# MarcioCerqueira/RealTimeDepthDiffusion

Hardware: AMD Instinct MI355X
Metric: Mpixel-iterations/s (solver sweep) (higher is better)
Workload: dtype f32

## Files before the change

### realtimedepthdiffusion_amd/csrc/persist_sync.hpp

```cpp
#pragma once
#include <hip/hip_runtime.h>

namespace rtdd {

constexpr int kSyncStatus = 0, kSyncWithhold = 1, kSyncLimit = 2, kSyncNonLocal = 3 , kSyncFailedSeq = 4,
              kSyncConfirmPtr = 6 , kSyncWild = 8, kSyncFlags = 32, kSyncMaxTiles = 1024, kSyncFlagStride = 64;
constexpr int kSyncWords = kSyncFlags + kSyncMaxTiles * kSyncFlagStride;
constexpr unsigned long long kDefaultPollLimit = 20000000ull;
constexpr unsigned long long kArrivalPollLimit = 150000ull;

constexpr float kWildDepth = 0x1p100f;

#ifdef __HIPCC__
__device__ __forceinline__ bool depth_is_wild(float d) { return !(__builtin_fabsf(d) < kWildDepth); }
__device__ __forceinline__ int load_wild_word(const int *sync_words) { return sync_words[kSyncWild]; }
__device__ __forceinline__ bool solve_is_dead(int *sync_words, int seq, bool first) {
    if (!sync_words) return false;
    if (__hip_atomic_load(&sync_words[kSyncStatus], __ATOMIC_RELAXED, __HIP_MEMORY_SCOPE_AGENT) == 0) {
        if (first && seq != 0) {
            int *confirm = *(int *const *)(sync_words + kSyncConfirmPtr);
            if (confirm) __hip_atomic_store(confirm, seq, __ATOMIC_RELAXED, __HIP_MEMORY_SCOPE_SYSTEM);
        }
        return false;
    }
    if (first && __hip_atomic_load(&sync_words[kSyncFailedSeq], __ATOMIC_RELAXED, __HIP_MEMORY_SCOPE_AGENT) == 0)
        __hip_atomic_store(&sync_words[kSyncFailedSeq], seq, __ATOMIC_RELAXED, __HIP_MEMORY_SCOPE_AGENT);
    return true;
}

__device__ __forceinline__ int exchange_poll_offset(int tid, int bx, int by, int gx, int gy, int tile_base) {
    const int pw = tid >> 6, pl = tid & 63;
    if (pw != 0 || pl >= 9 || pl == 4) return -1;
    const int nx = bx + pl % 3 - 1, ny = by + pl / 3 - 1;
    if (nx < 0 || ny < 0 || nx >= gx || ny >= gy) return -1;
    return (kSyncFlags + (tile_base + ny * gx + nx) * kSyncFlagStride) * (int)sizeof(int);
}

__device__ __forceinline__ int load_flag_at(const int *base, unsigned off) {
    int v;
    asm volatile("global_load_dword %0, %1, %2 sc1\n\ts_waitcnt vmcnt(0)" : "=v"(v) : "v"(off), "s"(base) : "memory");
    return v;
}

template <bool ACQUIRE = true, bool ARRIVAL = false>
__device__ __forceinline__ bool exchange_wait_at(int *sync_words, int *dead_lds, int tid, int tile_id, int poll_off, int value, int tile_base = 0) {
    int *flags = sync_words + kSyncFlags + tile_base * kSyncFlagStride;
    if (tid == 0 && __hip_atomic_load(&sync_words[kSyncWithhold], __ATOMIC_RELAXED, __HIP_MEMORY_SCOPE_AGENT) != tile_id + 1)
        __hip_atomic_store(&flags[tile_id * kSyncFlagStride], value, __ATOMIC_RELAXED, __HIP_MEMORY_SCOPE_AGENT);
    if (poll_off >= 0) {
        unsigned long long t0 = 0, limit = 0;
        unsigned spins = 0;
        while (load_flag_at(sync_words, (unsigned)poll_off) - value < 0) {
            __builtin_amdgcn_s_sleep(4);
            if ((++spins & 63u) == 0) {
                const unsigned long long now = __builtin_amdgcn_s_memrealtime();
                if (t0 == 0) {
                    t0 = now;
                    const int l = __hip_atomic_load(&sync_words[kSyncLimit], __ATOMIC_RELAXED, __HIP_MEMORY_SCOPE_AGENT);
                    limit = l > 0 ? (unsigned long long)l : kDefaultPollLimit;
                    if (ARRIVAL && limit > kArrivalPollLimit) limit = kArrivalPollLimit;
                }
                const bool failed = __hip_atomic_load(&sync_words[kSyncStatus], __ATOMIC_RELAXED, __HIP_MEMORY_SCOPE_AGENT) != 0;
                if (failed || now - t0 > limit) {
                    if (!failed) __hip_atomic_store(&sync_words[kSyncStatus], 1, __ATOMIC_RELAXED, __HIP_MEMORY_SCOPE_AGENT);
                    __hip_atomic_store(dead_lds, 1, __ATOMIC_RELAXED, __HIP_MEMORY_SCOPE_WORKGROUP);
                    break;
                }
            }
        }
    }
    if (ACQUIRE && tid < 64) { __builtin_amdgcn_fence(__ATOMIC_ACQUIRE, "agent"); asm volatile("s_waitcnt vmcnt(0)" ::: "memory"); }
    if (!ACQUIRE && tid < 64) asm volatile("s_waitcnt vmcnt(0)" ::: "memory");
    __syncthreads();
    return __hip_atomic_load(dead_lds, __ATOMIC_RELAXED, __HIP_MEMORY_SCOPE_WORKGROUP) != 0;
}

template <bool ACQUIRE = true, bool ARRIVAL = false>
__device__ __forceinline__ bool exchange_wait(int *sync_words, int *dead_lds, int tid, int tile_id, int bx, int by, int gx, int gy, int value, int tile_base = 0) {
    return exchange_wait_at<ACQUIRE, ARRIVAL>(sync_words, dead_lds, tid, tile_id, exchange_poll_offset(tid, bx, by, gx, gy, tile_base), value, tile_base);
}

#endif

}
```

### realtimedepthdiffusion_amd/csrc/rbgs_blocked.hip

```cpp
#include <type_traits>

#include "rtdd_internal.hpp"
#include "persist_sync.hpp"
#include "sweep_common.hpp"

namespace rtdd {
namespace {

__device__ __forceinline__ float from_prev_lane(float v) {
    return __int_as_float(__builtin_amdgcn_update_dpp(0, __float_as_int(v), 0x138, 0xF, 0xF, true));
}
__device__ __forceinline__ float from_next_lane(float v) {
    return __int_as_float(__builtin_amdgcn_update_dpp(0, __float_as_int(v), 0x130, 0xF, 0xF, true));
}
__device__ __forceinline__ float div3(float n, float d, float y) {
    const float q0 = n * y;
    const float r = __builtin_fmaf(-d, q0, n);
    return __builtin_fmaf(r, y, q0);
}


__device__ __forceinline__ void store_sc1(float4 *p, float4 v) {
    typedef float f4v __attribute__((ext_vector_type(4)));
    const f4v t = {v.x, v.y, v.z, v.w};
// ... 58 lines not shown
            wr[g][i] = (in && x0 + i + 1 < cols) ? lut[mv[i] & 255] : 0.0f;
            wd[g][i] = (in && y + 1 < rows) ? lut[(mv[i] >> 8) & 255] : 0.0f;
            if (!in || (mv[i] & kMetaDirichlet)) dirichlet |= 1u << (g * 4 + i);
        }
        const float w = from_prev_lane(wr[g][3]);
        wl0[g] = (lx > 0 && x0 > 0) ? w : 0.0f;
    }
    {
        const int y = y0 - 1;
        uint4 m = make_uint4(0, 0, 0, 0);
        const bool ok = colok && y >= 0 && y + 1 < rows;
        if (ok) m = *(const uint4 *)(M + (size_t)y * ip + x0);
        const uint32_t mv[4] = {m.x, m.y, m.z, m.w};
#pragma unroll
        for (int i = 0; i < 4; i++) wu0[i] = (ok && x0 + i < cols) ? lut[(mv[i] >> 8) & 255] : 0.0f;
    }
#pragma unroll
    for (int g = 0; g < G; g++)
#pragma unroll
        for (int i = 0; i < 4; i++) {
            const float wl = i == 0 ? wl0[g] : wr[g][i - 1];
            const float wu = g == 0 ? wu0[i] : wd[g - 1][i];
            float c = 0.0f;
            c += wl; c += wr[g][i]; c += wu; c += wd[g][i];
            cnt[g][i] = c == 0.0f ? 1.0f : c;
            rcp[g][i] = rcp_rn(cnt[g][i]);
            unsafe |= cnt[g][i] < 0x1p-126f;
        }
    const bool wave_unsafe = __builtin_amdgcn_ballot_w64(unsafe) != 0 || wild_word == wild_seq;

    constexpr uint32_t kTinyT = 2u * 0x0D800000u - 1u;
    const int wv = tid >> 6, nwv = (int)blockDim.x >> 6;
    const int flag_idx = (tid & 63) == 0 ? (wv > 0 ? wv - 1 : wv) : (wv < nwv - 1 ? wv + 1 : wv);
    auto publish = [&](int h, int buf) {
        *(f4r *)&edge[buf][tr][0][lx] = a[0];
        *(f4r *)&edge[buf][tr][1][lx] = a[G - 1];
        __hip_atomic_store(&published[wv], h + 1, __ATOMIC_RELEASE, __HIP_MEMORY_SCOPE_WORKGROUP);
    };
    auto half = [&](int h, auto fast, auto col, bool last_of_block) {
        constexpr bool FAST = decltype(fast)::value;
        constexpr int C = decltype(col)::value;
        for (;;) {
            const int f = __hip_atomic_load(&published[flag_idx], __ATOMIC_RELAXED, __HIP_MEMORY_SCOPE_WORKGROUP);
            if (__builtin_amdgcn_ballot_w64(f < h + 1) == 0) break;
            __builtin_amdgcn_s_sleep(1);
        }
        __builtin_amdgcn_fence(__ATOMIC_ACQUIRE, "workgroup");
        float4 up4 = edge[C][tr > 0 ? tr - 1 : 0][tr > 0 ? 1 : 0][lx];
        float4 dn4 = edge[C][tr < ntr - 1 ? tr + 1 : tr][tr < ntr - 1 ? 0 : 1][lx];
        if (!FAST) { if (tr == 0) up4 = make_float4(0, 0, 0, 0); if (tr == ntr - 1) dn4 = make_float4(0, 0, 0, 0); }
        const float up[4] = {up4.x, up4.y, up4.z, up4.w}, dn[4] = {dn4.x, dn4.y, dn4.z, dn4.w};
        float xl0[G], xr3[G];
        auto wsum = [&](int g, int i) {
            const float xl = i == 0 ? xl0[g] : a[g][i - 1];
            const float xr = i == 3 ? xr3[g] : a[g][i + 1];
            const float xu = g == 0 ? up[i] : a[g - 1][i];
            const float xd = g == G - 1 ? dn[i] : a[g + 1][i];
            const float wl = i == 0 ? wl0[g] : wr[g][i - 1];
            const float wu = g == 0 ? wu0[i] : wd[g - 1][i];
            float sum = 0.0f;
            sum = CONTRACT ? __builtin_fmaf(wl, xl, sum) : sum + wl * xl;
            sum = CONTRACT ? __builtin_fmaf(wr[g][i], xr, sum) : sum + wr[g][i] * xr;
            sum = CONTRACT ? __builtin_fmaf(wu, xu, sum) : sum + wu * xu;
            sum = CONTRACT ? __builtin_fmaf(wd[g][i], xd, sum) : sum + wd[g][i] * xd;
            return sum;
        };
        auto group = [&](auto pick) {
            float q[G][4];
            uint32_t tmin = 0xFFFFFFFFu;
#pragma unroll
            for (int g = 0; g < G; g++) {
                if (!pick(g)) continue;
                if (((g + 0) & 1) == C) { xl0[g] = from_prev_lane(a[g][3]); if (!FAST && lx == 0) xl0[g] = 0.0f; }
                if (((g + 3) & 1) == C) { xr3[g] = from_next_lane(a[g][0]); if (!FAST && lx == LX - 1) xr3[g] = 0.0f; }
#pragma unroll
                for (int i = 0; i < 4; i++) {
                    if (((g + i) & 1) != C) continue;
                    const float sum = wsum(g, i);
                    if (FAST) { q[g][i] = div3(sum, cnt[g][i], rcp[g][i]); tmin = min(tmin, (__float_as_uint(sum) << 1) + 0xFFFFFFFFu); }
                    else q[g][i] = sum / cnt[g][i];
                }
            }
            if (FAST && __builtin_expect(__builtin_amdgcn_ballot_w64(tmin < kTinyT) != 0, 0)) {
                bool suspect = false;
#pragma unroll
                for (int g = 0; g < G; g++) {
                    if (!pick(g)) continue;
#pragma unroll
                    for (int i = 0; i < 4; i++) {
                        if (((g + i) & 1) != C) continue;
                        bool s;
                        q[g][i] = div_tiny(wsum(g, i), cnt[g][i], rcp[g][i], s);
                        suspect |= s;
                    }
                }
                if (__builtin_expect(__builtin_amdgcn_ballot_w64(suspect) != 0, 0)) {
#pragma unroll
                    for (int g = 0; g < G; g++) {
                        if (!pick(g)) continue;
#pragma unroll
                        for (int i = 0; i < 4; i++) if (((g + i) & 1) == C) q[g][i] = wsum(g, i) / cnt[g][i];
                    }
                }
            }
#pragma unroll
            for (int g = 0; g < G; g++) {
                if (!pick(g)) continue;
#pragma unroll
                for (int i = 0; i < 4; i++) {
                    if (((g + i) & 1) != C) continue;
                    const float x = a[g][i];
                    float r = __builtin_amdgcn_fmed3f(q[g][i], 0.0f, 255.0f);
                    if (SOR) { r = CONTRACT ? __builtin_fmaf(omega, r - x, x) : x + omega * (r - x); r = __builtin_amdgcn_fmed3f(r, 0.0f, 255.0f); }
                    a[g][i] = (dirichlet >> (g * 4 + i)) & 1u ? x : r;
                }
            }
        };
        __builtin_amdgcn_s_setprio(1);
        group([](int g) { return g == 0 || g == G - 1; });
        if (!last_of_block) publish(h + 1, C ^ 1);
        __builtin_amdgcn_s_setprio(0);
        group([](int g) { return g != 0 && g != G - 1; });
    };

    const int tile_id = by * gx + bx;
    int h = 0, s = 0, blk = 0;
    for (;; blk++) {
        const int s_end = min(s + block_sweeps, nsweeps);
        publish(h, 0);
        using C0 = std::integral_constant<int, 0>; using C1 = std::integral_constant<int, 1>;
        for (; s < s_end; s++) {
            if (!wave_unsafe) { half(h, std::true_type{}, C0{}, false); half(h + 1, std::true_type{}, C1{}, s + 1 >= s_end); }
            else { half(h, std::false_type{}, C0{}, false); half(h + 1, std::false_type{}, C1{}, s + 1 >= s_end); }
            h += 2;
        }
        if (!PERSIST || s >= nsweeps) break;
        float *Ex = (blk & 1) ? X : Y;
        int tid_x = tid;
        asm volatile("" : "+v"(tid_x));
        const int lx = tid_x % LX, tr = tid_x / LX;
        const int x0 = bx * TW - hx + 4 * lx, y0 = by * TH - hy + tr * G;
        const bool colok = x0 >= 0 && x0 < cols;
        const bool xin = colok && 4 * lx >= hx && 4 * lx < EW - hx;
#pragma unroll
        for (int g = 0; g < G; g++) {
            const int y = y0 + g, ty = tr * G + g;
            const bool central = xin && ty >= hy && ty < eh - hy && y < rows;
            const bool band = ty < 2 * hy || ty >= eh - 2 * hy || 4 * lx < 2 * hx || 4 * lx >= EW - 2 * hx;
            if (central && band) store_sc1((float4 *)(Ex + (size_t)y * ip + x0), make_float4(a[g][0], a[g][1], a[g][2], a[g][3]));
        }
        asm volatile("s_waitcnt vmcnt(0)" ::: "memory");
        __syncthreads();
#ifndef RTDD_EXCHANGE_ACQUIRE
#define RTDD_EXCHANGE_ACQUIRE 0
#endif
        if (exchange_wait<RTDD_EXCHANGE_ACQUIRE != 0>(sync_words, &dead_s, tid, tile_id, bx, by, gx, gy, flag_base + blk + 1)) return;
#if RTDD_EXCHANGE_ACQUIRE
#pragma unroll
        for (int g = 0; g < G; g++) {
            const int y = y0 + g, ty = tr * G + g;
            const bool central = xin && ty >= hy && ty < eh - hy;
            if (colok && y >= 0 && y < rows && !central) {
                const float4 v = *(const float4 *)(Ex + (size_t)y * ip + x0);
                const float xv[4] = {v.x, v.y, v.z, v.w};
#pragma unroll
                for (int i = 0; i < 4; i++) a[g][i] = x0 + i < cols ? xv[i] : 0.0f;
            }
        }
#else
        typedef float f4v_t __attribute__((ext_vector_type(4)));
        f4v_t hv[G];
#pragma unroll
        for (int g = 0; g < G; g++) {
            const int y = y0 + g, ty = tr * G + g;
            const bool central = xin && ty >= hy && ty < eh - hy;
            hv[g] = a[g];
            if (colok && y >= 0 && y < rows && !central) {
                const float *q = Ex + (size_t)y * ip + x0;
                asm volatile("global_load_dwordx4 %0, %1, off sc1" : "+v"(hv[g]) : "v"(q) : "memory");
            }
        }
        static_assert(G == 4, "the wait below lists four registers");
        asm volatile("s_waitcnt vmcnt(0)" : "+v"(hv[0]), "+v"(hv[1]), "+v"(hv[2]), "+v"(hv[3]) :: "memory");
#pragma unroll
        for (int g = 0; g < G; g++) {
// ... 86 lines not shown
```

### realtimedepthdiffusion_amd/csrc/sweep_blocked.hip

```cpp
#include <type_traits>

#include "rtdd_internal.hpp"
#include "persist_sync.hpp"
#include "sweep_common.hpp"
#include "sweep_diag.hpp"

namespace rtdd {


template <bool CONTRACT, bool FAST>
__device__ __forceinline__ float relax(float xl, float xr, float xu, float xd, float wl, float wr, float wu, float wd,
                                       float cnt, float rcp, float x, float prev, float omega, float gamma) {
    float sum = 0.0f;
    sum = CONTRACT ? __builtin_fmaf(wl, xl, sum) : sum + wl * xl;
    sum = CONTRACT ? __builtin_fmaf(wr, xr, sum) : sum + wr * xr;
    sum = CONTRACT ? __builtin_fmaf(wu, xu, sum) : sum + wu * xu;
    sum = CONTRACT ? __builtin_fmaf(wd, xd, sum) : sum + wd * xd;
    float r;
    if (FAST) {
        r = div_tail(sum, cnt, rcp);
        const bool tiny = __builtin_fabsf(sum) < 0x1p-100f && sum != 0.0f;
        if (__builtin_expect(__builtin_amdgcn_ballot_w64(tiny) != 0, 0)) r = tiny ? sum / cnt : r;
    } else {
        r = sum / cnt;
    }
    r = __builtin_amdgcn_fmed3f(r, 0.0f, 255.0f);
    if (CONTRACT) return __builtin_fmaf(omega, __builtin_fmaf(gamma, r - x, x) - prev, prev);
    return (omega * (gamma * (r - x) + x - prev)) + prev;
}

template <int LX, int NT, int G, bool CONTRACT, bool PERSIST>
__global__ __launch_bounds__(NT, (NT >= 1024 || G <= 3 ? 4 : G <= 4 ? 3 : 2)) void k_sweep_blocked(float *Xk, float *Xm, float *Yk, float *Ym,
                                                      const uint32_t *__restrict__ M, const float *__restrict__ lut_g,
                                                      const float *__restrict__ omegas, int ip, int rows, int cols,
                                                      int hx, int hy, int nsweeps, float gamma,
                                                      int block_sweeps, int *sync_words, int gx, int gy, int xcd_tiles, int flag_base, size_t zPlane, int wild_seq) {
    constexpr int EW = 4 * LX, NTR = NT / LX;
    __shared__ float lut[257];
    __shared__ float4 edge[2][NTR][2][LX];
    __shared__ int published[NT / 64 + 1];
    __shared__ int dead_s;
    __shared__ int4 xrec[PERSIST ? NT : 1];

    int bx = blockIdx.x, by = blockIdx.y;
    if (xcd_tiles > 0) {
        const int t = ((int)blockIdx.x & 7) * xcd_tiles + ((int)blockIdx.x >> 3);
        if (t >= gx * gy) return;
        bx = t % gx; by = t / gx;
    }
    RTDD_Z(Xk, zPlane); RTDD_Z(Xm, zPlane); RTDD_Z(Yk, zPlane); RTDD_Z(Ym, zPlane); RTDD_Z(M, zPlane);
    RTDD_STAMP(0);
    __builtin_amdgcn_s_setprio(2);
    const int tid = threadIdx.x;
    const int lx = tid % LX, tr = tid / LX;
    const int ntr = (int)blockDim.x / LX;
    const int eh = ntr * G;
    const int TW = EW - 2 * hx, TH = eh - 2 * hy;
    const int x0 = bx * TW - hx + 4 * lx;
    const int y0 = by * TH - hy + tr * G;
    const bool colok = x0 >= 0 && x0 < cols;

    typedef float f4r __attribute__((ext_vector_type(4)));
    f4r a[G], b[G];
    float wr[G][4], wd[G][4], wl0[G], wu0[4], cnt[G][4], rcp[G][4];
    bool unsafe = false;
    uint32_t dirichlet = 0;

    const int wild_word = load_wild_word(sync_words);
    float4 vxr[G], vpr[G];
    uint4 mr[G], mup = make_uint4(0, 0, 0, 0);
#pragma unroll
    for (int g = 0; g < G; g++) {
        const int y = y0 + g;
        vxr[g] = make_float4(0, 0, 0, 0); vpr[g] = vxr[g]; mr[g] = make_uint4(0, 0, 0, 0);
        if (colok && y >= 0 && y < rows) {
            const size_t off = (size_t)y * ip + x0;
            vxr[g] = *(const float4 *)(Xk + off);
            vpr[g] = *(const float4 *)(Xm + off);
            mr[g] = *(const uint4 *)(M + off);
        }
    }
    if (colok && y0 - 1 >= 0 && y0 < rows) mup = *(const uint4 *)(M + (size_t)(y0 - 1) * ip + x0);
    for (int i = tid; i < 257; i += (int)blockDim.x) lut[i] = lut_g[i];
    if (tid <= NT / 64) published[tid] = 0;
    if (tid == 0) { dead_s = PERSIST && __hip_atomic_load(&sync_words[kSyncStatus], __ATOMIC_RELAXED, __HIP_MEMORY_SCOPE_AGENT) != 0; }
    const int ntiles = gx * gy, tile_base = (int)blockIdx.z * ntiles, tile_id = by * gx + bx;
    if (PERSIST) {
        if (exchange_wait_at<false, true>(sync_words, &dead_s, tid, tile_id, exchange_poll_offset(tid, bx, by, gx, gy, tile_base), flag_base, tile_base)) return;
    } else {
        __syncthreads();
    }

    RTDD_STAMP_LOADED(4);
    const int tx0 = bx * TW - hx, ty0 = by * TH - hy;
    const bool tile_inside = tx0 >= 0 && tx0 + EW < cols && ty0 >= 1 && ty0 + eh < rows;
#include "sweep_tile_setup.inc"
    if constexpr (PERSIST) {
        const bool xin = colok && 4 * lx >= hx && 4 * lx < EW - hx;
        uint32_t bits = 0;
#pragma unroll
        for (int g = 0; g < G; g++) {
            const int y = y0 + g, ty = tr * G + g;
            const bool central = xin && ty >= hy && ty < eh - hy;
            const bool band = ty < 2 * hy || ty >= eh - 2 * hy || 4 * lx < 2 * hx || 4 * lx >= EW - 2 * hx;
            const bool ok = colok && y >= 0 && y < rows;
            if (central && y < rows && band) bits |= 1u << g;
            if (ok && !central) bits |= 0x100u << g;
        }
        const int nv = min(max(cols - x0, 0), 4);
        bits |= (uint32_t)nv << 16;
        if (colok && nv < 4) bits |= 1u << 19;
        const uint32_t off0 = ((uint32_t)y0 * (uint32_t)ip + (uint32_t)x0) * 4u;
        xrec[tid] = make_int4((int)off0, (int)bits, exchange_poll_offset(tid, bx, by, gx, gy, tile_base), 0);
    }

    RTDD_STAMP(1);
    __builtin_amdgcn_s_setprio(0);
#include "sweep_tile_sweeps.inc"
    int s = 0, blk = 0;
    bool odd = false, dead = false;
    RTDD_XT_BEGIN;
    for (;; blk++) {
        const int s_end = min(s + block_sweeps, nsweeps);
        publish(a[0], a[G - 1], s, 0);
        using P0 = std::integral_constant<int, 0>; using P1 = std::integral_constant<int, 1>;
        if constexpr (!PERSIST) {
            if (!wave_unsafe) {
                for (; s + 1 < s_end; s += 2) {
                    sweep(a, b, s, std::true_type{}, false, P0{});
                    sweep(b, a, s + 1, std::true_type{}, s + 2 >= s_end, P1{});
                }
                if (s < s_end) { sweep(a, b, s, std::true_type{}, true, P0{}); s++; odd = true; }
            } else {
                for (; s + 1 < s_end; s += 2) {
                    sweep(a, b, s, std::false_type{}, false, P0{});
                    sweep(b, a, s + 1, std::false_type{}, s + 2 >= s_end, P1{});
                }
                if (s < s_end) { sweep(a, b, s, std::false_type{}, true, P0{}); s++; odd = true; }
            }
        } else {
            const int s_fast = wave_unsafe ? s : s_end;
            for (; s + 1 < s_fast; s += 2) {
                sweep(a, b, s, std::true_type{}, false, P0{});
                sweep(b, a, s + 1, std::true_type{}, s + 2 >= s_end, P1{});
            }
            if (s < s_fast) { sweep(a, b, s, std::true_type{}, true, P0{}); s++; odd = true; }
            while (s < s_end) {
                const bool single = s + 1 >= s_end;
                sweep(a, b, s, std::false_type{}, single, P0{});
                if (single) { s++; odd = true; break; }
                sweep(b, a, s + 1, std::false_type{}, s + 2 >= s_end, P1{});
                s += 2;
            }
        }
        if (!PERSIST || s >= nsweeps) break;
        RTDD_XT(0);

        {
            const float *Ek = (blk & 1) ? Xk : Yk, *Em = (blk & 1) ? Xm : Ym;
            int tid_x = tid;
            asm volatile("" : "+v"(tid_x));
            const int4 rec = xrec[tid_x];
            const uint32_t off0 = (uint32_t)rec.x, bits = (uint32_t)rec.y, pitch = (uint32_t)ip * 4u;
            RTDD_XT(5);
#pragma unroll
            for (int g = 0; g < G; g++) {
                if (bits & (1u << g)) {
                    store_sc1_at(Ek, off0 + g * pitch, a[g]);
                    store_sc1_at(Em, off0 + g * pitch, b[g]);
                }
            }
            asm volatile("s_waitcnt vmcnt(0)" ::: "memory");
            __syncthreads();
            RTDD_XT(1);
#ifndef RTDD_EXCHANGE_ACQUIRE
#define RTDD_EXCHANGE_ACQUIRE 0
#endif
            if (exchange_wait_at<RTDD_EXCHANGE_ACQUIRE != 0>(sync_words, &dead_s, tid, tile_id, rec.z, flag_base + blk + 1, tile_base)) { dead = true; break; }
            RTDD_XT(2);
            RTDD_XT(3);
#if RTDD_EXCHANGE_ACQUIRE
#pragma unroll
            for (int g = 0; g < G; g++) {
                if (bits & (0x100u << g)) {
                    a[g] = *(const f4r *)((const char *)Ek + (off0 + g * pitch));
                    b[g] = *(const f4r *)((const char *)Em + (off0 + g * pitch));
                }
            }
#else
            {
                uint32_t off[G];
                unsigned long long lanes[G];
#pragma unroll
                for (int g = 0; g < G; g++) { off[g] = off0 + g * pitch; lanes[g] = __builtin_amdgcn_ballot_w64((bits & (0x100u << g)) != 0); }
// ... 89 lines not shown
        dir[g] = in && (m & kMetaDirichlet);
        wl[g] = lane_from_prev(wr[g]);
    }
    {
        const int y = y0 - 1;
        const bool ok = colok && y >= 0 && y + 1 < rows;
        wu0 = ok ? lut[(mup >> 8) & 255] : 0.0f;
    }
#pragma unroll
    for (int g = 0; g < R; g++) {
        float c = 0.0f;
        c += wl[g]; c += wr[g]; c += g == 0 ? wu0 : wd[g - 1]; c += wd[g];
        cnt[g] = c == 0.0f ? 1.0f : c;
        rcp[g] = rcp_rn(cnt[g]);
        unsafe |= cnt[g] < 0x1p-126f;
    }
    const bool wave_unsafe = __builtin_amdgcn_ballot_w64(unsafe) != 0 || wild_word == wild_seq;
    constexpr uint32_t kTinyT = 2u * 0x0D800000u - 1u;
    const int up_w = wv > 0 ? wv - 1 : wv, dn_w = wv < nwv - 1 ? wv + 1 : wv;
    const int up_half = wv > 0 ? 1 : 0, dn_half = wv < nwv - 1 ? 0 : 1;
    auto publish = [&](int buf, float top, float bottom, int tag) {
        int *e = (int *)&edge[buf][wv][lane];
        asm volatile("" ::: "memory");
        e[0] = __float_as_int(top); e[2] = __float_as_int(bottom);
        asm volatile("" ::: "memory");
        __hip_atomic_store(&e[1], tag, __ATOMIC_RELAXED, __HIP_MEMORY_SCOPE_WORKGROUP);
        __hip_atomic_store(&e[3], tag, __ATOMIC_RELAXED, __HIP_MEMORY_SCOPE_WORKGROUP);
        asm volatile("" ::: "memory");
    };

    bool gone = false;
    const int tile_id_tl = by * gx + bx; (void)tile_id_tl;
    auto sweep = [&](float (&cur)[R], float (&oth)[R], int s, auto fast, bool last, auto parity) {
        constexpr bool FAST = decltype(fast)::value;
        constexpr int buf = decltype(parity)::value;
        float up, dn;
        RTDD_TL(0, s);
        {
            const long long *pu = (const long long *)&edge[buf][up_w][lane] + up_half, *pd = (const long long *)&edge[buf][dn_w][lane] + dn_half;
            auto read_both = [&]() {
                const long long u = __hip_atomic_load(pu, __ATOMIC_RELAXED, __HIP_MEMORY_SCOPE_WORKGROUP);
                const long long d = __hip_atomic_load(pd, __ATOMIC_RELAXED, __HIP_MEMORY_SCOPE_WORKGROUP);
                up = __int_as_float((int)u); dn = __int_as_float((int)d);
                const int tu = (int)(u >> 32), td = (int)(d >> 32);
                return __builtin_amdgcn_ballot_w64((tu < td ? tu : td) < s + 1) == 0;
            };
            if (__builtin_expect(!read_both(), 0)) {
                unsigned spins = 0;
                while (!gone) {
                    __builtin_amdgcn_s_sleep(1);
                    if (read_both()) break;
                    if (++spins > (1u << 22)) {
                        __hip_atomic_store(&sync_words[kSyncStatus], 2, __ATOMIC_RELAXED, __HIP_MEMORY_SCOPE_AGENT);
                        gone = true;
                    }
                }
                if (gone) { up = 0.0f; dn = 0.0f; }
            }
        }
        RTDD_TL_ROWS_IN_HAND(s);
        const float omega = omegas[s], gamma_v = gamma;
        auto wsum = [&](int g) {
            const float xl = lane_from_prev(cur[g]);
            const float xu = g == 0 ? up : cur[g - 1], xd = g == R - 1 ? dn : cur[g + 1];
            const float wu = g == 0 ? wu0 : wd[g - 1];
            float sum = 0.0f;
            sum = CONTRACT ? __builtin_fmaf(wl[g], xl, sum) : sum + wl[g] * xl;
            if (CONTRACT) {
                asm volatile("v_fmac_f32_dpp %0, %1, %2 wave_shl:1 row_mask:0xf bank_mask:0xf bound_ctrl:1" : "+v"(sum) : "v"(cur[g]), "v"(wr[g]));
            } else {
                sum = sum + wr[g] * lane_from_next(cur[g]);
            }
            sum = CONTRACT ? __builtin_fmaf(wu, xu, sum) : sum + wu * xu;
            sum = CONTRACT ? __builtin_fmaf(wd[g], xd, sum) : sum + wd[g] * xd;
            return sum;
        };
        auto pair = [&](int g0, int g1) {
            const float s0 = wsum(g0), s1 = wsum(g1);
            float q0, q1;
            if (FAST) {
                q0 = div_tail(s0, cnt[g0], rcp[g0]); q1 = div_tail(s1, cnt[g1], rcp[g1]);
                const uint32_t t0 = (__float_as_uint(s0) << 1) + 0xFFFFFFFFu, t1 = (__float_as_uint(s1) << 1) + 0xFFFFFFFFu;
                if (__builtin_expect(__builtin_amdgcn_ballot_w64((t0 < t1 ? t0 : t1) < kTinyT) != 0, 0)) {
                    bool u0, u1;
                    q0 = div_tiny(s0, cnt[g0], rcp[g0], u0); q1 = div_tiny(s1, cnt[g1], rcp[g1], u1);
                    if (__builtin_expect(__builtin_amdgcn_ballot_w64(u0 || u1) != 0, 0)) { q0 = s0 / cnt[g0]; q1 = s1 / cnt[g1]; }
                }
            } else { q0 = s0 / cnt[g0]; q1 = s1 / cnt[g1]; }
            const int gs[2] = {g0, g1}; const float qs[2] = {q0, q1};
#pragma unroll
            for (int k = 0; k < 2; k++) {
                const int g = gs[k];
                const float r = __builtin_amdgcn_fmed3f(qs[k], 0.0f, 255.0f);
                const float xc = cur[g], prev = oth[g];
                const float v = CONTRACT ? __builtin_fmaf(omega, __builtin_fmaf(gamma_v, r - xc, xc) - prev, prev)
                                         : (omega * (gamma_v * (r - xc) + xc - prev)) + prev;
                oth[g] = dir[g] ? xc : v;
            }
        };
        __builtin_amdgcn_s_setprio(1);
        pair(0, R - 1);
        if (!last) publish(buf ^ 1, oth[0], oth[R - 1], s + 2);
        __builtin_amdgcn_s_setprio(0);
        RTDD_TL(2, s);
        pair(1, 2);
        RTDD_TL(3, s);
    };

    publish(0, a[0], a[R - 1], 1);
    using P0 = std::integral_constant<int, 0>; using P1 = std::integral_constant<int, 1>;
    const int n = nsweeps;
    const int a0 = n + 2 - hy + R * wv, a1 = n - 2 - R * wv + eh - hy;
    const int active_until = min(n - 1, min(a0, a1));
    int s = 0;
    bool odd = false;
    if (!wave_unsafe) {
        for (; s + 1 < n && s + 1 <= active_until; s += 2) { sweep(a, b, s, std::true_type{}, false, P0{}); sweep(b, a, s + 1, std::true_type{}, s + 2 >= n, P1{}); }
        if (s < n && s <= active_until) { sweep(a, b, s, std::true_type{}, s + 1 >= n, P0{}); odd = true; }
    } else {
        for (; s + 1 < n && s + 1 <= active_until; s += 2) { sweep(a, b, s, std::false_type{}, false, P0{}); sweep(b, a, s + 1, std::false_type{}, s + 2 >= n, P1{}); }
        if (s < n && s <= active_until) { sweep(a, b, s, std::false_type{}, s + 1 >= n, P0{}); odd = true; }
    }
    if (active_until < n - 1) {
        for (int bf = 0; bf < 2; bf++) {
            int *e = (int *)&edge[bf][wv][lane];
            __hip_atomic_store(&e[1], 0x7FFFFFFF, __ATOMIC_RELAXED, __HIP_MEMORY_SCOPE_WORKGROUP);
            __hip_atomic_store(&e[3], 0x7FFFFFFF, __ATOMIC_RELAXED, __HIP_MEMORY_SCOPE_WORKGROUP);
        }
        return;
    }
    const bool xin = colok && lane >= hx && lane < 64 - hx;
#pragma unroll
    for (int g = 0; g < R; g++) {
        const int y = y0 + g, ty = R * wv + g;
        if (xin && ty >= hy && ty < eh - hy && y < rows) {
            const size_t off = (size_t)y * ip + x;
            Yk[off] = odd ? b[g] : a[g];
            Ym[off] = odd ? a[g] : b[g];
        }
    }
}

struct TileCfg { int lx, nt, g; };
static const TileCfg kTiles[] = {{0, 0, 0}, {16, 256, 4}, {32, 512, 4}, {32, 1024, 4}, {32, 1024, 3}, {32, 512, 3}, {16, 512, 3}, {16, 256, 3}, {32, 1024, 2},
                                 {16, 1024, 1}, {16, 512, 2}, {32, 1024, 1}, {32, 768, 4}, {32, 512, 6},
                                 {16, 1024, 1} ,
                                 {16, 512, 1} , {16, 768, 1} };
constexpr int kNumTiles = 16;
static inline bool is_col_tile(int tile) { return tile >= 14; }
static inline int tile_rows(int tile, int nthreads) { return nthreads / kTiles[tile].lx * kTiles[tile].g; }

template <typename K>
static bool fits_one_per_cu(K kernel, int nthreads) {
    int nb = 0;
    return hipOccupancyMaxActiveBlocksPerMultiprocessor(&nb, kernel, nthreads, 0) == hipSuccess && nb >= 1;
}

template <int LX, int NT, int G>
static bool persistent_possible(rtdd_ctx *ctx, int tile, int nthreads) {
    signed char &c = ctx->persist_fit[tile][ctx->opt.fp_contract ? 1 : 0];
    if (c < 0) c = ctx->opt.fp_contract ? fits_one_per_cu(k_sweep_blocked<LX, NT, G, true, true>, nthreads) : fits_one_per_cu(k_sweep_blocked<LX, NT, G, false, true>, nthreads);
    return c == 1;
}

template <int LX, int NT, int G>
static void launch_cfg(rtdd_ctx *ctx, dim3 grid, int xcd_tiles, int nthreads, float *Xk, float *Xm, float *Yk, float *Ym, const uint32_t *M,
                       const float *omegas, int ip, int rows, int cols, int hx, int hy, int n, float gamma, int block_sweeps, int flag_base, size_t zPlane, int images) {
    const bool persist = block_sweeps < n;
    const dim3 launch_grid = xcd_tiles > 0 ? dim3(8 * xcd_tiles, 1, images) : dim3(grid.x, grid.y, images);
// ... 181 lines not shown
```

### realtimedepthdiffusion_amd/csrc/sweep_common.hpp

```cpp
#pragma once
#include <hip/hip_runtime.h>

namespace rtdd {

__device__ __forceinline__ float lane_from_prev(float v) {
    return __int_as_float(__builtin_amdgcn_update_dpp(0, __float_as_int(v), 0x138, 0xF, 0xF, true));
}
__device__ __forceinline__ float lane_from_next(float v) {
    return __int_as_float(__builtin_amdgcn_update_dpp(0, __float_as_int(v), 0x130, 0xF, 0xF, true));
}

__device__ __forceinline__ float lds_from_prev(int prev4, float v) { return __int_as_float(__builtin_amdgcn_ds_bpermute(prev4, __float_as_int(v))); }
__device__ __forceinline__ float lds_from_next(int prev4, float v) { return __int_as_float(__builtin_amdgcn_ds_bpermute(prev4 + 8, __float_as_int(v))); }

typedef float f4v_t __attribute__((ext_vector_type(4)));
__device__ __forceinline__ void store_sc1_at(const float *base, uint32_t off, f4v_t v) {
    asm volatile("global_store_dwordx4 %0, %1, %2 sc1\n\ts_nop 1" ::"v"(off), "v"(v), "s"(base) : "memory");
}
#define RTDD_HALO_ROW(n) "s_and_b64 exec, %[sv], %[m" #n "]\n\tglobal_load_dwordx4 %[a" #n "], %[o" #n "], %[bk] sc1\n\tglobal_load_dwordx4 %[b" #n "], %[o" #n "], %[bm] sc1\n\t"
#define RTDD_HALO_OUT(n) [a##n] "+v"(a[n]), [b##n] "+v"(b[n])
#define RTDD_HALO_IN(n) [o##n] "v"(off[n]), [m##n] "s"(mask[n])
#define RTDD_HALO_ASM(rows, outs, ins) asm volatile("s_mov_b64 %[sv], exec\n\t" rows "s_mov_b64 exec, %[sv]\n\ts_waitcnt vmcnt(0)" : outs, [sv] "=&s"(sv) : ins, [bk] "s"(bk), [bm] "s"(bm) : "memory", "scc")
#define RTDD_C ,
template <int G>
__device__ __forceinline__ void load_halo_rows_sc1(f4v_t (&a)[G], f4v_t (&b)[G], const float *bk, const float *bm, const uint32_t (&off)[G], const unsigned long long (&mask)[G]) {
    unsigned long long sv;
    if constexpr (G == 1) RTDD_HALO_ASM(RTDD_HALO_ROW(0), RTDD_HALO_OUT(0), RTDD_HALO_IN(0));
    else if constexpr (G == 2) RTDD_HALO_ASM(RTDD_HALO_ROW(0) RTDD_HALO_ROW(1), RTDD_HALO_OUT(0) RTDD_C RTDD_HALO_OUT(1), RTDD_HALO_IN(0) RTDD_C RTDD_HALO_IN(1));
    else if constexpr (G == 3) RTDD_HALO_ASM(RTDD_HALO_ROW(0) RTDD_HALO_ROW(1) RTDD_HALO_ROW(2), RTDD_HALO_OUT(0) RTDD_C RTDD_HALO_OUT(1) RTDD_C RTDD_HALO_OUT(2),
                                             RTDD_HALO_IN(0) RTDD_C RTDD_HALO_IN(1) RTDD_C RTDD_HALO_IN(2));
    else if constexpr (G == 4) RTDD_HALO_ASM(RTDD_HALO_ROW(0) RTDD_HALO_ROW(1) RTDD_HALO_ROW(2) RTDD_HALO_ROW(3), RTDD_HALO_OUT(0) RTDD_C RTDD_HALO_OUT(1) RTDD_C RTDD_HALO_OUT(2) RTDD_C RTDD_HALO_OUT(3),
                                             RTDD_HALO_IN(0) RTDD_C RTDD_HALO_IN(1) RTDD_C RTDD_HALO_IN(2) RTDD_C RTDD_HALO_IN(3));
    else {
        static_assert(G == 6, "add a statement for this G");
        RTDD_HALO_ASM(RTDD_HALO_ROW(0) RTDD_HALO_ROW(1) RTDD_HALO_ROW(2) RTDD_HALO_ROW(3) RTDD_HALO_ROW(4) RTDD_HALO_ROW(5),
                      RTDD_HALO_OUT(0) RTDD_C RTDD_HALO_OUT(1) RTDD_C RTDD_HALO_OUT(2) RTDD_C RTDD_HALO_OUT(3) RTDD_C RTDD_HALO_OUT(4) RTDD_C RTDD_HALO_OUT(5),
                      RTDD_HALO_IN(0) RTDD_C RTDD_HALO_IN(1) RTDD_C RTDD_HALO_IN(2) RTDD_C RTDD_HALO_IN(3) RTDD_C RTDD_HALO_IN(4) RTDD_C RTDD_HALO_IN(5));
    }
}
#undef RTDD_C
#undef RTDD_HALO_ASM
#undef RTDD_HALO_IN
#undef RTDD_HALO_OUT
#undef RTDD_HALO_ROW

__device__ __forceinline__ void store_result(float4 *p, float4 v) { *p = v; }

__device__ __forceinline__ float div_tail(float n, float d, float y) {
    const float q0 = n * y;
    const float r = __builtin_fmaf(-d, q0, n);
    return __builtin_fmaf(r, y, q0);
}

__device__ __forceinline__ float div_tiny(float n, float d, float y, bool &suspect) {
    const bool tiny = __builtin_fabsf(n) < 0x1p-100f;
    const float up = tiny ? 0x1p64f : 1.0f, down = tiny ? 0x1p-64f : 1.0f;
    const float N = n * up;
    const float Q = div_tail(N, d, y);
    const float q = Q * down;
    suspect = __builtin_fabsf(__builtin_fmaf(q, -up, Q)) == 0x1p-86f;
    return q;
}

__device__ __forceinline__ float rcp_rn(float d) {
    const float y0 = __builtin_amdgcn_rcpf(d);
    return __builtin_fmaf(__builtin_fmaf(-d, y0, 1.0f), y0, y0);
}

__device__ __forceinline__ void masked_fmac4(float &o0, float &o1, float &o2, float &o3, float w, float t0, float t1, float t2, float t3,
                                             unsigned long long m0, unsigned long long m1, unsigned long long m2, unsigned long long m3) {
    unsigned long long entry;
    asm("s_and_saveexec_b64 %[e], %[m0]\n\tv_fmac_f32_e32 %[o0], %[w], %[t0]\n\t"
        "s_and_b64 exec, %[e], %[m1]\n\tv_fmac_f32_e32 %[o1], %[w], %[t1]\n\t"
        "s_and_b64 exec, %[e], %[m2]\n\tv_fmac_f32_e32 %[o2], %[w], %[t2]\n\t"
        "s_and_b64 exec, %[e], %[m3]\n\tv_fmac_f32_e32 %[o3], %[w], %[t3]\n\t"
        "s_mov_b64 exec, %[e]"
        : [o0] "+v"(o0), [o1] "+v"(o1), [o2] "+v"(o2), [o3] "+v"(o3), [e] "=&s"(entry)
        : [w] "v"(w), [t0] "v"(t0), [t1] "v"(t1), [t2] "v"(t2), [t3] "v"(t3), [m0] "s"(m0), [m1] "s"(m1), [m2] "s"(m2), [m3] "s"(m3)
        : "scc");
}
__device__ __forceinline__ void masked_add4(float &o0, float &o1, float &o2, float &o3, float p0, float p1, float p2, float p3,
                                            unsigned long long m0, unsigned long long m1, unsigned long long m2, unsigned long long m3) {
    unsigned long long entry;
    asm("s_and_saveexec_b64 %[e], %[m0]\n\tv_add_f32_e32 %[o0], %[p0], %[o0]\n\t"
        "s_and_b64 exec, %[e], %[m1]\n\tv_add_f32_e32 %[o1], %[p1], %[o1]\n\t"
        "s_and_b64 exec, %[e], %[m2]\n\tv_add_f32_e32 %[o2], %[p2], %[o2]\n\t"
        "s_and_b64 exec, %[e], %[m3]\n\tv_add_f32_e32 %[o3], %[p3], %[o3]\n\t"
        "s_mov_b64 exec, %[e]"
        : [o0] "+v"(o0), [o1] "+v"(o1), [o2] "+v"(o2), [o3] "+v"(o3), [e] "=&s"(entry)
        : [p0] "v"(p0), [p1] "v"(p1), [p2] "v"(p2), [p3] "v"(p3), [m0] "s"(m0), [m1] "s"(m1), [m2] "s"(m2), [m3] "s"(m3)
        : "scc");
}

}
```

### realtimedepthdiffusion_amd/csrc/sweep_tile_sweeps.inc

```
    constexpr uint32_t kTinyT = 2u * 0x0D800000u - 1u;
    const int prev4 = (((int)threadIdx.x + 63) & 63) * 4;
    const int wv = tid >> 6, nwv = (int)blockDim.x >> 6;
    const int tile_id_tl = by * gx + bx; (void)tile_id_tl;
    auto publish = [&](const f4r &top, const f4r &bottom, int sweep_no, int buf) {
        *(f4r *)&edge[buf][tr][0][lx] = top;
        if (G > 1) *(f4r *)&edge[buf][tr][1][lx] = bottom;
        if (!PERSIST) {
            asm volatile("" ::: "memory");
            __hip_atomic_store(&published[wv], sweep_no + 1, __ATOMIC_RELAXED, __HIP_MEMORY_SCOPE_WORKGROUP);
            asm volatile("" ::: "memory");
        } else {
            __hip_atomic_store(&published[wv], sweep_no + 1, __ATOMIC_RELEASE, __HIP_MEMORY_SCOPE_WORKGROUP);
        }
    };
    unsigned lds_spins = 0;
    bool gone = false;
    auto await = [&](int sweep_no) {
        if (gone) return;
        const int idx = (tid & 63) == 0 ? (wv > 0 ? wv - 1 : wv) : (wv < nwv - 1 ? wv + 1 : wv);
        auto there = [&]() { return __builtin_amdgcn_ballot_w64(__hip_atomic_load(&published[idx], __ATOMIC_RELAXED, __HIP_MEMORY_SCOPE_WORKGROUP) < sweep_no + 1) == 0; };
        if (__builtin_expect(!there(), 0)) {
            for (;;) {
                __builtin_amdgcn_s_sleep(1);
                if (there()) break;
                if ((++lds_spins & 1023u) == 0) {
                    if (__hip_atomic_load(&dead_s, __ATOMIC_RELAXED, __HIP_MEMORY_SCOPE_WORKGROUP) != 0) { gone = true; break; }
                    if (lds_spins > (1u << 22)) {
                        __hip_atomic_store(&sync_words[kSyncStatus], 2, __ATOMIC_RELAXED, __HIP_MEMORY_SCOPE_AGENT);
                        __hip_atomic_store(&dead_s, 1, __ATOMIC_RELAXED, __HIP_MEMORY_SCOPE_WORKGROUP);
                        gone = true; break;
                    }
                }
            }
        }
        __builtin_amdgcn_fence(__ATOMIC_ACQUIRE, "workgroup");
    };
    auto sweep = [&](f4r (&cur)[G], f4r (&oth)[G], int s, auto fast, bool last_of_block, auto parity) {
        constexpr bool FAST = decltype(fast)::value;
        constexpr int buf = decltype(parity)::value;
        RTDD_TL(0, s);
        float xl0[G], xr3[G];
        auto shifts = [&](int g) {
            xl0[g] = lds_from_prev(prev4, wr[g][3] * cur[g][3]); xr3[g] = lds_from_next(prev4, cur[g][0]);
            if (!FAST) { xl0[g] = lx == 0 ? 0.0f : xl0[g]; xr3[g] = lx == LX - 1 ? 0.0f : xr3[g]; }
        };
        shifts(0); if (G > 1) shifts(G - 1);
        await(s);
        float4 up4 = edge[buf][tr > 0 ? tr - 1 : 0][G > 1 && tr > 0 ? 1 : 0][lx];
        float4 dn4 = edge[buf][tr < ntr - 1 ? tr + 1 : tr][G == 1 || tr < ntr - 1 ? 0 : 1][lx];
        if (!FAST) { if (tr == 0) up4 = make_float4(0, 0, 0, 0); if (tr == ntr - 1) dn4 = make_float4(0, 0, 0, 0); }
        const float up[4] = {up4.x, up4.y, up4.z, up4.w}, dn[4] = {dn4.x, dn4.y, dn4.z, dn4.w};
        RTDD_TL_ROWS_IN_HAND(s);
        float omega_v = omegas[s], gamma_v = gamma;
        asm volatile("" : "+v"(omega_v), "+v"(gamma_v));
        auto wsum = [&](int g, int i) {
            const float xl = i == 0 ? xl0[g] : cur[g][i - 1];
            const float xr = i == 3 ? xr3[g] : cur[g][i + 1];
            const float xu = g == 0 ? up[i] : cur[g - 1][i];
            const float xd = g == G - 1 ? dn[i] : cur[g + 1][i];
            const float wu = g == 0 ? wu0[i] : wd[g - 1][i];
            float sum = i == 0 ? 0.0f + xl0[g] : (CONTRACT ? __builtin_fmaf(wr[g][i - 1], xl, 0.0f) : 0.0f + wr[g][i - 1] * xl);
            sum = CONTRACT ? __builtin_fmaf(wr[g][i], xr, sum) : sum + wr[g][i] * xr;
            sum = CONTRACT ? __builtin_fmaf(wu, xu, sum) : sum + wu * xu;
            sum = CONTRACT ? __builtin_fmaf(wd[g][i], xd, sum) : sum + wd[g][i] * xd;
            return sum;
        };
        auto group = [&](auto pick) {
            float q[G][4], sums[G][4];
            uint32_t tmin = 0xFFFFFFFFu;
#pragma unroll
            for (int g = 0; g < G; g++) {
                if (!pick(g)) continue;
                uint32_t t[4];
#pragma unroll
                for (int i = 0; i < 4; i++) {
                    const float sum = sums[g][i] = wsum(g, i);
                    if (FAST) { q[g][i] = div_tail(sum, cnt[g][i], rcp[g][i]); t[i] = (__float_as_uint(sum) << 1) + 0xFFFFFFFFu; }
                    else q[g][i] = sum / cnt[g][i];
                }
                if (FAST) { tmin = min(min(tmin, t[0]), t[1]); tmin = min(min(tmin, t[2]), t[3]); }
            }
            if (FAST && __builtin_expect(__builtin_amdgcn_ballot_w64(tmin < kTinyT) != 0, 0)) {
                auto sum_of = [&](int g, int i) { return PERSIST ? sums[g][i] : wsum(g, i); };
                bool suspect = false;
#pragma unroll
                for (int g = 0; g < G; g++) {
                    if (!pick(g)) continue;
#pragma unroll
                    for (int i = 0; i < 4; i++) {
                        bool s;
                        q[g][i] = div_tiny(sum_of(g, i), cnt[g][i], rcp[g][i], s);
                        suspect |= s;
                    }
                }
                if (__builtin_expect(__builtin_amdgcn_ballot_w64(suspect) != 0, 0)) {
#pragma unroll
                    for (int g = 0; g < G; g++) {
                        if (!pick(g)) continue;
#pragma unroll
                        for (int i = 0; i < 4; i++) q[g][i] = sum_of(g, i) / cnt[g][i];
                    }
                }
            }
#pragma unroll
            for (int g = 0; g < G; g++) {
                if (!pick(g)) continue;
                float t[4], o[4];
#pragma unroll
                for (int i = 0; i < 4; i++) {
                    const float r = __builtin_amdgcn_fmed3f(q[g][i], 0.0f, 255.0f);
                    const float x = cur[g][i];
                    o[i] = oth[g][i];
                    t[i] = (CONTRACT ? __builtin_fmaf(gamma_v, r - x, x) : gamma_v * (r - x) + x) - o[i];
                    if (!CONTRACT) t[i] = omega_v * t[i];
                }
                if (CONTRACT) masked_fmac4(o[0], o[1], o[2], o[3], omega_v, t[0], t[1], t[2], t[3], free_mask[g][0], free_mask[g][1], free_mask[g][2], free_mask[g][3]);
                else masked_add4(o[0], o[1], o[2], o[3], t[0], t[1], t[2], t[3], free_mask[g][0], free_mask[g][1], free_mask[g][2], free_mask[g][3]);
#pragma unroll
                for (int i = 0; i < 4; i++) oth[g][i] = o[i];
            }
        };
        __builtin_amdgcn_s_setprio(1);
        group([](int g) { return g == 0; });
#pragma unroll
        for (int gi = 1; gi < G - 1; gi++) shifts(gi);
        if (G > 1) group([](int g) { return g == G - 1; });
        if (!last_of_block) publish(oth[0], oth[G - 1], s + 1, buf ^ 1);
        __builtin_amdgcn_s_setprio(0);
        RTDD_TL(2, s);
#pragma unroll
        for (int gi = 1; gi < G - 1; gi++) group([gi](int g) { return g == gi; });
        if constexpr (PERSIST && G == 1) asm volatile("" : "+v"(oth[0]));
        RTDD_TL(3, s);
    };
```

Baseline: 1.598 million.

## Simplify tiny-sum division, add s_nop padding before sync asm, branchless mask bits

Rewrites div_tiny so the scaled residual step is folded into the division, which removes the suspect flag and the extra ballot/IEEE-divide fallback on tiny sums. It also inserts s_nop padding before the flag polling load, the sc1 store and the halo-load asm blocks, and turns the persistent-tile mask-bit setup into branchless bitwise logic. The division change shortens a rarely taken slow path but could change rounding on tiny inputs. The nops add a few cycles per use, apparently to avoid hazards or to space out memory instructions.

```diff
diff --git a/realtimedepthdiffusion_amd/csrc/persist_sync.hpp b/realtimedepthdiffusion_amd/csrc/persist_sync.hpp
--- a/realtimedepthdiffusion_amd/csrc/persist_sync.hpp
+++ b/realtimedepthdiffusion_amd/csrc/persist_sync.hpp
@@ -38,7 +38,7 @@
 
 __device__ __forceinline__ int load_flag_at(const int *base, unsigned off) {
     int v;
-    asm volatile("global_load_dword %0, %1, %2 sc1\n\ts_waitcnt vmcnt(0)" : "=v"(v) : "v"(off), "s"(base) : "memory");
+    asm volatile("s_nop 4\n\tglobal_load_dword %0, %1, %2 sc1\n\ts_waitcnt vmcnt(0)" : "=v"(v) : "v"(off), "s"(base) : "memory");
     return v;
 }
 
diff --git a/realtimedepthdiffusion_amd/csrc/rbgs_blocked.hip b/realtimedepthdiffusion_amd/csrc/rbgs_blocked.hip
--- a/realtimedepthdiffusion_amd/csrc/rbgs_blocked.hip
+++ b/realtimedepthdiffusion_amd/csrc/rbgs_blocked.hip
@@ -164,25 +164,11 @@
                 }
             }
             if (FAST && __builtin_expect(__builtin_amdgcn_ballot_w64(tmin < kTinyT) != 0, 0)) {
-                bool suspect = false;
 #pragma unroll
                 for (int g = 0; g < G; g++) {
                     if (!pick(g)) continue;
 #pragma unroll
-                    for (int i = 0; i < 4; i++) {
-                        if (((g + i) & 1) != C) continue;
-                        bool s;
-                        q[g][i] = div_tiny(wsum(g, i), cnt[g][i], rcp[g][i], s);
-                        suspect |= s;
-                    }
-                }
-                if (__builtin_expect(__builtin_amdgcn_ballot_w64(suspect) != 0, 0)) {
-#pragma unroll
-                    for (int g = 0; g < G; g++) {
-                        if (!pick(g)) continue;
-#pragma unroll
-                        for (int i = 0; i < 4; i++) if (((g + i) & 1) == C) q[g][i] = wsum(g, i) / cnt[g][i];
-                    }
+                    for (int i = 0; i < 4; i++) if (((g + i) & 1) == C) q[g][i] = div_tiny(wsum(g, i), cnt[g][i], rcp[g][i]);
                 }
             }
 #pragma unroll
diff --git a/realtimedepthdiffusion_amd/csrc/sweep_blocked.hip b/realtimedepthdiffusion_amd/csrc/sweep_blocked.hip
--- a/realtimedepthdiffusion_amd/csrc/sweep_blocked.hip
+++ b/realtimedepthdiffusion_amd/csrc/sweep_blocked.hip
@@ -96,20 +96,20 @@
     const bool tile_inside = tx0 >= 0 && tx0 + EW < cols && ty0 >= 1 && ty0 + eh < rows;
 #include "sweep_tile_setup.inc"
     if constexpr (PERSIST) {
-        const bool xin = colok && 4 * lx >= hx && 4 * lx < EW - hx;
+        const bool xin = colok & (4 * lx >= hx) & (4 * lx < EW - hx);
         uint32_t bits = 0;
 #pragma unroll
         for (int g = 0; g < G; g++) {
             const int y = y0 + g, ty = tr * G + g;
-            const bool central = xin && ty >= hy && ty < eh - hy;
-            const bool band = ty < 2 * hy || ty >= eh - 2 * hy || 4 * lx < 2 * hx || 4 * lx >= EW - 2 * hx;
-            const bool ok = colok && y >= 0 && y < rows;
-            if (central && y < rows && band) bits |= 1u << g;
-            if (ok && !central) bits |= 0x100u << g;
+            const bool central = xin & (ty >= hy) & (ty < eh - hy);
+            const bool band = (ty < 2 * hy) | (ty >= eh - 2 * hy) | (4 * lx < 2 * hx) | (4 * lx >= EW - 2 * hx);
+            const bool ok = colok & (y >= 0) & (y < rows);
+            bits |= (uint32_t)(central & (y < rows) & band) << g;
+            bits |= (uint32_t)(ok & !central) << (8 + g);
         }
         const int nv = min(max(cols - x0, 0), 4);
         bits |= (uint32_t)nv << 16;
-        if (colok && nv < 4) bits |= 1u << 19;
+        bits |= (uint32_t)(colok & (nv < 4)) << 19;
         const uint32_t off0 = ((uint32_t)y0 * (uint32_t)ip + (uint32_t)x0) * 4u;
         xrec[tid] = make_int4((int)off0, (int)bits, exchange_poll_offset(tid, bx, by, gx, gy, tile_base), 0);
     }
@@ -365,9 +365,7 @@
                 q0 = div_tail(s0, cnt[g0], rcp[g0]); q1 = div_tail(s1, cnt[g1], rcp[g1]);
                 const uint32_t t0 = (__float_as_uint(s0) << 1) + 0xFFFFFFFFu, t1 = (__float_as_uint(s1) << 1) + 0xFFFFFFFFu;
                 if (__builtin_expect(__builtin_amdgcn_ballot_w64((t0 < t1 ? t0 : t1) < kTinyT) != 0, 0)) {
-                    bool u0, u1;
-                    q0 = div_tiny(s0, cnt[g0], rcp[g0], u0); q1 = div_tiny(s1, cnt[g1], rcp[g1], u1);
-                    if (__builtin_expect(__builtin_amdgcn_ballot_w64(u0 || u1) != 0, 0)) { q0 = s0 / cnt[g0]; q1 = s1 / cnt[g1]; }
+                    q0 = div_tiny(s0, cnt[g0], rcp[g0]); q1 = div_tiny(s1, cnt[g1], rcp[g1]);
                 }
             } else { q0 = s0 / cnt[g0]; q1 = s1 / cnt[g1]; }
             const int gs[2] = {g0, g1}; const float qs[2] = {q0, q1};
diff --git a/realtimedepthdiffusion_amd/csrc/sweep_common.hpp b/realtimedepthdiffusion_amd/csrc/sweep_common.hpp
--- a/realtimedepthdiffusion_amd/csrc/sweep_common.hpp
+++ b/realtimedepthdiffusion_amd/csrc/sweep_common.hpp
@@ -15,12 +15,12 @@
 
 typedef float f4v_t __attribute__((ext_vector_type(4)));
 __device__ __forceinline__ void store_sc1_at(const float *base, uint32_t off, f4v_t v) {
-    asm volatile("global_store_dwordx4 %0, %1, %2 sc1\n\ts_nop 1" ::"v"(off), "v"(v), "s"(base) : "memory");
+    asm volatile("s_nop 4\n\tglobal_store_dwordx4 %0, %1, %2 sc1\n\ts_nop 1" ::"v"(off), "v"(v), "s"(base) : "memory");
 }
 #define RTDD_HALO_ROW(n) "s_and_b64 exec, %[sv], %[m" #n "]\n\tglobal_load_dwordx4 %[a" #n "], %[o" #n "], %[bk] sc1\n\tglobal_load_dwordx4 %[b" #n "], %[o" #n "], %[bm] sc1\n\t"
 #define RTDD_HALO_OUT(n) [a##n] "+v"(a[n]), [b##n] "+v"(b[n])
 #define RTDD_HALO_IN(n) [o##n] "v"(off[n]), [m##n] "s"(mask[n])
-#define RTDD_HALO_ASM(rows, outs, ins) asm volatile("s_mov_b64 %[sv], exec\n\t" rows "s_mov_b64 exec, %[sv]\n\ts_waitcnt vmcnt(0)" : outs, [sv] "=&s"(sv) : ins, [bk] "s"(bk), [bm] "s"(bm) : "memory", "scc")
+#define RTDD_HALO_ASM(rows, outs, ins) asm volatile("s_nop 2\n\ts_mov_b64 %[sv], exec\n\t" rows "s_mov_b64 exec, %[sv]\n\ts_waitcnt vmcnt(0)" : outs, [sv] "=&s"(sv) : ins, [bk] "s"(bk), [bm] "s"(bm) : "memory", "scc")
 #define RTDD_C ,
 template <int G>
 __device__ __forceinline__ void load_halo_rows_sc1(f4v_t (&a)[G], f4v_t (&b)[G], const float *bk, const float *bm, const uint32_t (&off)[G], const unsigned long long (&mask)[G]) {
@@ -52,14 +52,13 @@
     return __builtin_fmaf(r, y, q0);
 }
 
-__device__ __forceinline__ float div_tiny(float n, float d, float y, bool &suspect) {
+__device__ __forceinline__ float div_tiny(float n, float d, float y) {
     const bool tiny = __builtin_fabsf(n) < 0x1p-100f;
     const float up = tiny ? 0x1p64f : 1.0f, down = tiny ? 0x1p-64f : 1.0f;
     const float N = n * up;
-    const float Q = div_tail(N, d, y);
-    const float q = Q * down;
-    suspect = __builtin_fabsf(__builtin_fmaf(q, -up, Q)) == 0x1p-86f;
-    return q;
+    const float qd = (N * y) * down;
+    const float R = __builtin_fmaf(-d, qd * up, N);
+    return __builtin_fmaf(R, y * down, qd);
 }
 
 __device__ __forceinline__ float rcp_rn(float d) {
diff --git a/realtimedepthdiffusion_amd/csrc/sweep_tile_sweeps.inc b/realtimedepthdiffusion_amd/csrc/sweep_tile_sweeps.inc
--- a/realtimedepthdiffusion_amd/csrc/sweep_tile_sweeps.inc
+++ b/realtimedepthdiffusion_amd/csrc/sweep_tile_sweeps.inc
@@ -82,24 +82,11 @@
             }
             if (FAST && __builtin_expect(__builtin_amdgcn_ballot_w64(tmin < kTinyT) != 0, 0)) {
                 auto sum_of = [&](int g, int i) { return PERSIST ? sums[g][i] : wsum(g, i); };
-                bool suspect = false;
 #pragma unroll
                 for (int g = 0; g < G; g++) {
                     if (!pick(g)) continue;
 #pragma unroll
-                    for (int i = 0; i < 4; i++) {
-                        bool s;
-                        q[g][i] = div_tiny(sum_of(g, i), cnt[g][i], rcp[g][i], s);
-                        suspect |= s;
-                    }
-                }
-                if (__builtin_expect(__builtin_amdgcn_ballot_w64(suspect) != 0, 0)) {
-#pragma unroll
-                    for (int g = 0; g < G; g++) {
-                        if (!pick(g)) continue;
-#pragma unroll
-                        for (int i = 0; i < 4; i++) q[g][i] = sum_of(g, i) / cnt[g][i];
-                    }
+                    for (int i = 0; i < 4; i++) q[g][i] = div_tiny(sum_of(g, i), cnt[g][i], rcp[g][i]);
                 }
             }
 #pragma unroll
```

Result: faster. 1.646 million, median of 6 (+3.0%).
